# GTEC-UDC/roskfpos

Hardware: AMD Instinct MI355X
Metric: EKF predict+update steps/s at 65536 tags x 8 anchors; RMS pos err vs CPU ref (higher is better)
Workload: dtype f64 arithmetic; f64 state and covariance, f32/int32 measurements in HBM (KFPOS_STORE_MIXED)

## Files before the change

### __graft_entry__.py

```python
from __future__ import annotations

import os
import shutil
import subprocess
import sys

ROOT = os.path.dirname(os.path.abspath(__file__))
CSRC = os.path.join(ROOT, "roskfpos_amd", "csrc")
HIP_LIB = os.path.join(CSRC, "libkfpos_hip.so")
ADAPTOR_DEMO = os.path.join(CSRC, "kfpos_replay")


def _stale(target, sources):
    if not os.path.exists(target):
        return True
    mt = os.path.getmtime(target)
    return any(os.path.getmtime(s) > mt for s in sources if os.path.exists(s))


def build(force: bool = False) -> None:
    jobs = str(min(8, os.cpu_count() or 1))
    res = subprocess.run(["make", "-s", "-j", jobs, "-C", CSRC] + (["-B"] if force else []) + ["all"],
                         capture_output=True, text=True)
    if res.returncode != 0:
        sys.stderr.write(res.stdout + res.stderr)
        raise subprocess.CalledProcessError(res.returncode, res.args)
    res = subprocess.run(["make", "-s", "-C", CSRC, "check"], capture_output=True, text=True)
    if res.returncode != 0:
        sys.stderr.write(res.stdout + res.stderr)
        if os.path.exists(HIP_LIB):
            os.remove(HIP_LIB)
        raise RuntimeError("a build-time performance rule is broken (scratch inside a loop / a kernel lost its second "
                           "wavefront per SIMD / the 9-state epoch loop waits for a memory operation just issued): " + (res.stdout + res.stderr).strip())
    subprocess.check_call(["make", "-s", "-C", os.path.join(ROOT, "oracle")] + (["-B"] if force else []))
    import glob
    core_headers = sorted(glob.glob(os.path.join(CSRC, "kfpos_core*.h"))) + [os.path.join(CSRC, "kfpos_p48.h")]
    emu_dir = os.path.join(ROOT, "tests", "emu")
    emu_so = os.path.join(emu_dir, "libkfpos_emu.so")
    if force or _stale(emu_so, [os.path.join(emu_dir, "kfpos_emu.cpp")] + core_headers):
        subprocess.check_call(["g++", "-O2", "-std=c++17", "-fPIC", "-shared", "-Wno-unknown-pragmas",
                               "-o", emu_so, os.path.join(emu_dir, "kfpos_emu.cpp")])
    fake_dir = os.path.join(ROOT, "tests", "fake_rccl")
    fake_so = os.path.join(fake_dir, "libfake_rccl.so")
    if force or _stale(fake_so, [os.path.join(fake_dir, "fake_rccl.cpp")]):
        subprocess.check_call([shutil.which("hipcc") or "/opt/rocm/bin/hipcc", "-O2", "-std=c++17", "-shared", "-fPIC",
                               "-o", fake_so, os.path.join(fake_dir, "fake_rccl.cpp"), "-lrt"])
    if ROOT not in sys.path:
        sys.path.insert(0, ROOT)
    import roskfpos_amd
    from roskfpos_amd import capi
    capi.load()


def smoke() -> None:
    if ROOT not in sys.path:
        sys.path.insert(0, ROOT)
# ... 34 lines not shown
```

### roskfpos_amd/csrc/kfpos_core.h

```cpp
#ifndef KFPOS_CORE_H
#define KFPOS_CORE_H

#include <math.h>
#include <stdint.h>

#ifndef KFPOS_HD
#define KFPOS_HD
#endif
#define KFPOS_FN KFPOS_HD inline __attribute__((always_inline))
#if defined(__clang__)
#define KFPOS_UNROLL _Pragma("unroll")
#define KFPOS_NOUNROLL _Pragma("nounroll")
#else
#define KFPOS_UNROLL
#define KFPOS_NOUNROLL
#endif

#if defined(__HIP_DEVICE_COMPILE__)
#define KFPOS_WAVE_ALL(pred) (__all((pred) ? 1 : 0) != 0)
#else
#define KFPOS_WAVE_ALL(pred) (pred)
#endif

namespace kfpos {

enum : uint32_t {
    ST_UPDATE_SKIPPED = 0x01u,
    ST_ML_FALLBACK    = 0x02u,
    ST_FEW_RANGES     = 0x04u,
    ST_ML_INIT        = 0x08u,
    ST_NOT_STARTED    = 0x10u,
    ST_NONFINITE      = 0x20u,
    ST_SKIPPED        = 0x40u,
};
enum : uint32_t { FL_STARTED = 1u, FL_HAS_IMU = 2u };

KFPOS_FN uint32_t pack_status(uint32_t flags, int gain_iters, int ml_iters, int ignored) {
    const uint32_t g = gain_iters > 255 ? 255u : (uint32_t)gain_iters;
    const uint32_t m = ml_iters > 255 ? 255u : (uint32_t)ml_iters;
    return flags | (g << 8) | (m << 16) | ((uint32_t)(ignored + 1) << 24);
}

KFPOS_FN double kf_rcp(double x) {
#if defined(__HIP_DEVICE_COMPILE__)
    double y = __builtin_amdgcn_rcp(x);
    double e = __builtin_fma(-x, y, 1.0);
    y = __builtin_fma(y, e, y);
    e = __builtin_fma(-x, y, 1.0);
    return __builtin_fma(y, e, y);
#else
    return 1.0 / x;
#endif
}
KFPOS_FN double kf_fma(double a, double b, double c) {
#if defined(__HIP_DEVICE_COMPILE__)
    return __builtin_fma(a, b, c);
#else
    return a * b + c;
#endif
}
KFPOS_FN int kf_opaque_zero() {
    int z = 0;
#if defined(__HIP_DEVICE_COMPILE__)
    asm volatile("" : "+v"(z));
#endif
    return z;
}
KFPOS_FN int kf_ctz64(uint64_t m) {
#if defined(__HIP_DEVICE_COMPILE__)
    return __ffsll((unsigned long long)m) - 1;
#else
    return __builtin_ctzll(m);
#endif
}
KFPOS_FN double kf_rsqrt(double x) {
#if defined(__HIP_DEVICE_COMPILE__)
    double y = __builtin_amdgcn_rsq(x);
    const double h = 0.5 * x;
    double e = __builtin_fma(-h * y, y, 0.5);
    y = __builtin_fma(y, e, y);
    e = __builtin_fma(-h * y, y, 0.5);
    return __builtin_fma(y, e, y);
#else
    return 1.0 / sqrt(x);
#endif
}
KFPOS_FN void kf_sqrt_rsqrt(double x, double &d, double &invd) {
#if defined(__HIP_DEVICE_COMPILE__)
    invd = kf_rsqrt(x);
    const double s = x * invd;
// ... 14 lines not shown
    invd = y;
#else
    d = sqrt(x);
    invd = 1.0 / d;
#endif
}

KFPOS_FN double kf_mm_to_m(int32_t mm) {
#if defined(__HIP_DEVICE_COMPILE__)
    const double x = (double)mm;
    const double q = x * 0.001;
    const double r = __builtin_fma(-q, 1000.0, x);
    return __builtin_fma(r, 0.001, q);
#else
    return (double)mm / 1000;
#endif
}

KFPOS_FN bool rel_change_below(double cost, double c, double tol) {
    const double lhs = fabs(cost - c), rhs = tol * cost;
    const bool clear = cost > 0.0 && fabs(lhs - rhs) > 1e-13 * rhs;
    if (KFPOS_WAVE_ALL(clear)) return lhs < rhs;
    return lhs / cost < tol;
}

KFPOS_FN bool rel_change_above(double cost, double c, double tol) {
    const double lhs = fabs(cost - c), rhs = tol * cost;
    const bool clear = cost > 0.0 && fabs(lhs - rhs) > 1e-13 * rhs;
    if (KFPOS_WAVE_ALL(clear)) return lhs > rhs;
    return lhs / cost > tol;
}

KFPOS_FN double stdmax(double a, double b) { return (a < b) ? b : a; }

template <int N, bool SYMM>
struct Cov {
    static constexpr int SZ = SYMM ? N * (N + 1) / 2 : N * N;
    double a[SZ];
    KFPOS_HD static constexpr int idx(int i, int j) {
        return SYMM ? (i <= j ? i * N - i * (i - 1) / 2 + (j - i) : j * N - j * (j - 1) / 2 + (i - j))
                    : i * N + j;
    }
    KFPOS_HD double operator()(int i, int j) const { return a[idx(i, j)]; }
    KFPOS_HD double &operator()(int i, int j) { return a[idx(i, j)]; }
};

// ... 252 lines not shown
```

### roskfpos_amd/csrc/kfpos_core_imu9.h

```cpp
#ifndef KFPOS_CORE_IMU9_H
#define KFPOS_CORE_IMU9_H

namespace kfpos {

constexpr double INFO_FORM_MIN_PIVOT = 1e-7;

struct Tag9 {
    double pos[3], vel[3];
    Cov<9, true> P;
};
struct Imu {
    bool has;
    double acc[3];
    double *ci;
    int ci_stride;
    KFPOS_HD double Wi(int k) const { return ci[(6 + k) * ci_stride]; }
};

KFPOS_FN void imu_whitener(const double s[9], double *ci, int ci_stride) {
    double c00, c11, c22, i00, i11, i22;
    kf_sqrt_rsqrt(s[0], c00, i00);
    const double c10 = s[3] * i00, c20 = s[6] * i00;
    kf_sqrt_rsqrt(s[4] - c10 * c10, c11, i11);
    const double c21 = (s[7] - c20 * c10) * i11;
// ... 407 lines not shown
            u0 += gx * yw; u1 += gy * yw; u2 += gz * yw;
            const double wx = w * gx, wy = w * gy, wz = w * gz;
            m0 += wx * gx; m1 += wx * gy; m2 += wx * gz;
            m3 += wy * gy; m4 += wy * gz; m5 += wz * gz;
        });
        s.c = c;
        s.m[0] = m0; s.m[1] = m1; s.m[2] = m2; s.m[3] = m3; s.m[4] = m4; s.m[5] = m5;
        s.u[0] = u0; s.u[1] = u1; s.u[2] = u2;
    }
}

KFPOS_FN void iekf9_spread_reads() {
#if defined(__HIP_DEVICE_COMPILE__)
    KFPOS_UNROLL
    for (int k = 0; k < 20; ++k) {
        __builtin_amdgcn_sched_group_barrier(0x100, 1, 0);
        __builtin_amdgcn_sched_group_barrier(0x002, 10, 0);
    }
#endif
}
struct Iekf9Parked {
    double binv[21], wi[6];
};
template <bool EVERY_TRIP>
KFPOS_FN void iekf9_fetch(const double *binv, int binv_stride, const Imu &imu, Iekf9Parked &pk) {
    const int z = EVERY_TRIP ? kf_opaque_zero() : 0;
    KFPOS_UNROLL
    for (int k = 0; k < 21; ++k) pk.binv[k] = binv[k * binv_stride + z];
    KFPOS_UNROLL
    for (int k = 0; k < 6; ++k) pk.wi[k] = imu.ci[(6 + k) * imu.ci_stride + z];
}
template <bool DIAG>
KFPOS_FN bool iekf9_pass(const double xhat[9], const Iekf9Parked &pk, const Imu &imu, double tol,
                         const Sweep9 &sw, Iekf9Iter &it, Iekf9Out &o) {
    const double *ve = it.ve;
    const double acc[3] = {xhat[6] + ve[3], xhat[7] + ve[4], xhat[8] + ve[5]};
    double c = it.qd + sw.c;
    const double m0 = sw.m[0], m1 = sw.m[1], m2 = sw.m[2], m3 = sw.m[3], m4 = sw.m[4], m5 = sw.m[5];
    const double m[6] = {m0, m1, m2, m3, m4, m5};
    double u[6] = {sw.u[0] + (m0 * ve[0] + m1 * ve[1] + m2 * ve[2]), sw.u[1] + (m1 * ve[0] + m3 * ve[1] + m4 * ve[2]),
                   sw.u[2] + (m2 * ve[0] + m4 * ve[1] + m5 * ve[2]), 0.0, 0.0, 0.0};
    double ma[6] = {0, 0, 0, 0, 0, 0};
    if (imu.has) {
        const double ya[3] = {imu.acc[0] - acc[0], imu.acc[1] - acc[1], imu.acc[2] - acc[2]};
        const double va[3] = {ya[0] + acc[0] * ve[3], ya[1] + acc[1] * ve[4], ya[2] + acc[2] * ve[5]};
        if constexpr (DIAG) {
            const double wd[3] = {pk.wi[0], pk.wi[3], pk.wi[5]};
            KFPOS_UNROLL
            for (int i = 0; i < 3; ++i) {
                const double wy = wd[i] * ya[i];
                c += ya[i] * wy;
                u[3 + i] = acc[i] * (wd[i] * va[i]);
            }
            ma[0] = acc[0] * acc[0] * wd[0]; ma[3] = acc[1] * acc[1] * wd[1]; ma[5] = acc[2] * acc[2] * wd[2];
        } else {
            const double wm[3][3] = {{pk.wi[0], pk.wi[1], pk.wi[2]},
                                     {pk.wi[1], pk.wi[3], pk.wi[4]},
                                     {pk.wi[2], pk.wi[4], pk.wi[5]}};
            KFPOS_UNROLL
            for (int i = 0; i < 3; ++i) {
                const double wy = wm[i][0] * ya[0] + wm[i][1] * ya[1] + wm[i][2] * ya[2];
                c += ya[i] * wy;
                u[3 + i] = acc[i] * (wm[i][0] * va[0] + wm[i][1] * va[1] + wm[i][2] * va[2]);
            }
            ma[0] = acc[0] * acc[0] * wm[0][0]; ma[1] = acc[0] * acc[1] * wm[0][1]; ma[2] = acc[0] * acc[2] * wm[0][2];
            ma[3] = acc[1] * acc[1] * wm[1][1]; ma[4] = acc[1] * acc[2] * wm[1][2]; ma[5] = acc[2] * acc[2] * wm[2][2];
        }
    }
    if (rel_change_below(it.cost, c, tol)) return false;
#ifdef KFPOS_EMU_ITER_TRACE
    kfpos_emu_iter_trace(o.gain_iters, ve, c);
#endif
    it.cost = c;
    KFPOS_UNROLL
    for (int k = 0; k < 6; ++k) o.mrlast[k] = m[k];
    o.dlast[0] = acc[0]; o.dlast[1] = acc[1]; o.dlast[2] = acc[2];

    Cov<6, true> K;
    KFPOS_UNROLL
    for (int k = 0; k < 21; ++k) K.a[k] = pk.binv[k];
    K(0, 0) += m[0]; K(0, 1) += m[1]; K(0, 2) += m[2]; K(1, 1) += m[3]; K(1, 2) += m[4]; K(2, 2) += m[5];
    K(3, 3) += ma[0]; K(4, 4) += ma[3]; K(5, 5) += ma[5];
    if constexpr (!DIAG) { K(3, 4) += ma[1]; K(3, 5) += ma[2]; K(4, 5) += ma[4]; }
    double v[6];
    sym6_solve(K, u, v);
    double *wl = it.wl;
    wl[0] = u[0] - (m[0] * v[0] + m[1] * v[1] + m[2] * v[2]);
    wl[1] = u[1] - (m[1] * v[0] + m[3] * v[1] + m[4] * v[2]);
    wl[2] = u[2] - (m[2] * v[0] + m[4] * v[1] + m[5] * v[2]);
    wl[3] = u[3] - (ma[0] * v[3] + ma[1] * v[4] + ma[2] * v[5]);
    wl[4] = u[4] - (ma[1] * v[3] + ma[3] * v[4] + ma[4] * v[5]);
    wl[5] = u[5] - (ma[2] * v[3] + ma[4] * v[4] + ma[5] * v[5]);
    double qd = 0.0;
    KFPOS_UNROLL
    for (int i = 0; i < 6; ++i) qd += wl[i] * v[i];
    it.qd = qd;
    KFPOS_UNROLL
    for (int i = 0; i < 6; ++i) it.ve[i] = v[i];
    o.gain_iters++;
    return true;
}

#if defined(__HIP_DEVICE_COMPILE__)
KFPOS_FN double lane_pull(double v, int src4) {
    const int lo = __builtin_amdgcn_ds_bpermute(src4, __double2loint(v));
    const int hi = __builtin_amdgcn_ds_bpermute(src4, __double2hiint(v));
    return __hiloint2double(hi, lo);
}
KFPOS_FN int nth_set_bit(uint64_t m, int n) {
    uint32_t w = (uint32_t)m;
    int base = 0;
    const int c0 = __popc(w);
    if (n >= c0) { n -= c0; w = (uint32_t)(m >> 32); base = 32; }
    KFPOS_UNROLL
    for (int width = 16; width >= 1; width >>= 1) {
        const uint32_t low = w & ((1u << width) - 1u);
        const int c = __popc(low);
        if (n >= c) { n -= c; w >>= width; base += width; }
        else w = low;
    }
    return base;
}

// ... 29 lines not shown
    ci.has = __builtin_amdgcn_ds_bpermute(src4, imu.has ? 1 : 0) != 0;
    KFPOS_UNROLL
    for (int k = 0; k < 3; ++k) ci.acc[k] = lane_pull(imu.acc[k], src4);
    ci.ci = imu.ci + (src - lane);
    ci.ci_stride = imu.ci_stride;
    double r4[4], w4[4];
    KFPOS_UNROLL
    for (int k = 0; k < 4; ++k) {
        const double r0 = lane_pull(sc.r[k], src4), r1 = lane_pull(sc.r[4 + k], src4);
        const double w0 = lane_pull(sc.w[k], src4), w1 = lane_pull(sc.w[4 + k], src4);
        r4[k] = h ? r1 : r0;
        w4[k] = h ? w1 : w0;
    }
    const double *cbinv = binv + (src - lane);
    const double *b4 = anchor_tab + 12 * h;
    const double b0[3] = {b4[0], b4[1], b4[2]};
    while (act) {
        double bb[12];
        const int z = kf_opaque_zero();
        bb[0] = b0[0]; bb[1] = b0[1]; bb[2] = b0[2];
        KFPOS_UNROLL
        for (int k = 3; k < 12; ++k) bb[k] = b4[k + z];
        Iekf9Parked pk;
        iekf9_fetch<true>(cbinv, binv_stride, ci, pk);
        const double p[3] = {xh[0] + ct.ve[0], xh[1] + ct.ve[1], xh[2] + ct.ve[2]};
        Sweep9 sw, other;
        iekf9_sweep4(p, r4, w4, bb, sw);
        other.c = dpp_exchange(sw.c, 0);
        KFPOS_UNROLL
        for (int k = 0; k < 6; ++k) other.m[k] = dpp_exchange(sw.m[k], 0);
        KFPOS_UNROLL
        for (int k = 0; k < 3; ++k) other.u[k] = dpp_exchange(sw.u[k], 0);
        sweep9_add(sw, other);
        iekf9_spread_reads();
        const bool more = iekf9_pass<DIAG>(xh, pk, ci, tol, sw, ct, co);
        act = more && co.gain_iters < max_steps;
    }
    const bool owner = (m >> lane) & 1ull;
    const int rank = __popcll(m & ((1ull << lane) - 1ull));
    const int from4 = (owner ? 2 * rank : lane) << 2;
    KFPOS_UNROLL
    for (int k = 0; k < 6; ++k) {
        const double a = lane_pull(ct.wl[k], from4), b = lane_pull(co.mrlast[k], from4);
        if (owner) { it.wl[k] = a; o.mrlast[k] = b; }
    }
    KFPOS_UNROLL
    for (int k = 0; k < 3; ++k) {
        const double a = lane_pull(co.dlast[k], from4);
        if (owner) o.dlast[k] = a;
    }
    const double cst = lane_pull(ct.cost, from4);
    const int gi = __builtin_amdgcn_ds_bpermute(from4, co.gain_iters);
    if (owner) { it.cost = cst; o.gain_iters = gi; }
}
#endif

template <bool DIAG, bool RANGING, bool ACC0 = false, class SC>
KFPOS_FN void iekf9_info(const double xhat[9], const double *binv, int binv_stride, SC &sc, const Params &pr,
                         const Imu &imu, int max_steps, double tol, Iekf9Out &o) {
    Iekf9Iter it;
    KFPOS_UNROLL
    for (int k = 0; k < 6; ++k) { it.ve[k] = 0.0; it.wl[k] = 0.0; o.mrlast[k] = 0.0; }
    it.qd = 0.0;
    it.cost = 1e20;
    o.dlast[0] = o.dlast[1] = o.dlast[2] = 0.0;
    o.gain_iters = 0;
#if defined(__HIP_DEVICE_COMPILE__)
    constexpr bool PAIRS = RANGING && SC::NA == 8 && SC::CHUNK == 0 && !SC::COOP;
    const bool pairs = PAIRS && pr.pair_anchor_tab && __builtin_amdgcn_ballot_w64(true) == ~0ull;
#endif
    bool more = true;
    int stop = max_steps;
#if defined(__HIP_DEVICE_COMPILE__)
    if (pairs) stop = 8 < max_steps ? 8 : max_steps;
#endif
    for (;;) {
        while (more && o.gain_iters < stop) {
            Iekf9Parked pk;
            iekf9_fetch<false>(binv, binv_stride, imu, pk);
            const double p[3] = {xhat[0] + it.ve[0], xhat[1] + it.ve[1], xhat[2] + it.ve[2]};
            Sweep9 sw;
            iekf9_sweep<RANGING>(p, sc, pr, sw);
            more = iekf9_pass<DIAG>(xhat, pk, imu, tol, sw, it, o);
        }
#if defined(__HIP_DEVICE_COMPILE__)
        if constexpr (PAIRS) {
            if (pairs) {
                const uint64_t m = __builtin_amdgcn_ballot_w64(more && o.gain_iters < max_steps);
                if (m == 0) break;
                if (__popcll(m) <= 32) {
                    iekf9_pairs<DIAG, ACC0>(m, xhat, binv, binv_stride, sc, pr.pair_anchor_tab, imu, max_steps, tol, it, o);
                    break;
                }
                stop = stop + 4 < max_steps ? stop + 4 : max_steps;
                continue;
            }
        }
#endif
        break;
    }
    KFPOS_UNROLL
    for (int k = 0; k < 6; ++k) o.w[k] = it.wl[k];
    o.cost = it.cost;
}

KFPOS_FN void cov_update9(Cov<9, true> &P, const double mr[6], const double d[3], const Imu &imu) {
// ... 12 lines not shown
            }
            pt[i] = v;
        }
        KFPOS_UNROLL
        for (int l = 0; l < 6; ++l) {
            const bool nz = (l < 3 && k < 3 && l >= k) || (l >= 3 && k >= 3 && l <= k);
            if (nz) s += L9(f, l, k) * pt[e9(l)];
        }
        const double is = kf_rcp(s);
        KFPOS_UNROLL
        for (int i = 0; i < 9; ++i) {
            const double pi = pt[i] * is;
            KFPOS_UNROLL
            for (int j = i; j < 9; ++j) P(i, j) -= pi * pt[j];
        }
    }
}

struct CovPark9 {
    double *a;
    int stride;
};

template <bool RANGING, class SC>
KFPOS_FN bool step_imu9_state(Tag9 &tg, SC &sc, const Params &pr, double dt, const Imu &imu, const CovPark9 &park,
                              bool diag, Iekf9Out &o, uint32_t &status) {
    constexpr bool has_ranging = RANGING;
    const int n_valid = has_ranging ? count_used(sc, pr, 0) : 0;
    if (!pr.use_init_pos && (isnan(tg.pos[0]) || isnan(tg.pos[1]))) {
        status = 0;
        if (!has_ranging) return false;
        status = ST_FEW_RANGES;
        if (n_valid < 4) return false;
        double p[3] = {1.0, 1.0, 4.0}, sse, c[6];
        set_weights_ml(sc, pr, 0ull);
        const int it = ml_estimate(p, sc, pr, 0, n_valid, sse);
        status = ST_UPDATE_SKIPPED;
        if (ml_covariance_throws(sc, pr, 0, n_valid, sse)) return false;
        if (!ml_covariance(p, sc, pr, sse, c)) return false;
        tg.pos[0] = p[0]; tg.pos[1] = p[1]; tg.pos[2] = p[2];
        tg.P(0, 0) = c[0]; tg.P(0, 1) = c[1]; tg.P(1, 1) = c[3];
        status = pack_status(ST_ML_INIT, 0, it, -1);
        return false;
    }
    const double c = dt * dt / 2;
    double xhat[9];
    KFPOS_UNROLL
    for (int k = 0; k < 3; ++k) {
        xhat[k] = tg.pos[k] + dt * tg.vel[k] + c * 0.0;
        xhat[3 + k] = tg.vel[k] + dt * 0.0;
        xhat[6 + k] = 0.0;
    }
    predict9(tg.P, dt, pr.jolt);
    Cov<6, true> B;
    KFPOS_UNROLL
    for (int i = 0; i < 6; ++i) {
        KFPOS_UNROLL
        for (int j = i; j < 6; ++j) B(i, j) = tg.P(e9(i), e9(j));
    }
    KFPOS_UNROLL
    for (int k = 0; k < 45; ++k) park.a[k * park.stride] = tg.P.a[k];
    double *binv = park.a + 45 * park.stride;
    const bool invertible = sym6_inverse(B, binv, park.stride, INFO_FORM_MIN_PIVOT);
    iekf9_weights(xhat, sc, pr, has_ranging, n_valid, o);
    if (o.flags & ST_UPDATE_SKIPPED) {
        KFPOS_UNROLL
        for (int k = 0; k < 45; ++k) tg.P.a[k] = park.a[k * park.stride];
        status = ST_UPDATE_SKIPPED;
        return false;
    }
    if (invertible) {
        if (diag) iekf9_info<true, RANGING, true>(xhat, binv, park.stride, sc, pr, imu, 20, 1e-4, o);
        else iekf9_info<false, RANGING, true>(xhat, binv, park.stride, sc, pr, imu, 20, 1e-4, o);
        KFPOS_UNROLL
        for (int k = 0; k < 45; ++k) tg.P.a[k] = park.a[k * park.stride];
    } else {
        KFPOS_UNROLL
        for (int k = 0; k < 45; ++k) tg.P.a[k] = park.a[k * park.stride];
        if (diag) iekf9<true, RANGING>(xhat, tg.P, sc, pr, imu, 20, 1e-4, o);
        else iekf9<false, RANGING>(xhat, tg.P, sc, pr, imu, 20, 1e-4, o);
    }
    KFPOS_UNROLL
    for (int i = 0; i < 6; ++i) {
        double v = 0.0;
        KFPOS_UNROLL
        for (int k = 0; k < 6; ++k) v += tg.P(i, e9(k)) * o.w[k];
        if (i < 3) tg.pos[i] = xhat[i] + v;
        else tg.vel[i - 3] = xhat[i] + v;
    }
    status = 0;
    return true;
}
KFPOS_FN uint32_t step_imu9_cov(Tag9 &tg, const Iekf9Out &o, const Imu &imu) {
    cov_update9(tg.P, o.mrlast, o.dlast, imu);
    return pack_status(o.flags, o.gain_iters, o.ml_iters, -1);
}
template <bool RANGING, class SC>
KFPOS_FN uint32_t step_imu9(Tag9 &tg, SC &sc, const Params &pr, double dt, const Imu &imu, const CovPark9 &park) {
    Iekf9Out o;
    uint32_t status;
    if (!step_imu9_state<RANGING>(tg, sc, pr, dt, imu, park, false, o, status)) return status;
    return step_imu9_cov(tg, o, imu);
// ... 22 lines not shown
```

### roskfpos_amd/csrc/kfpos_k_imu9.hip

```cpp
#include "kfpos_kernels.h"

namespace {

template <typename REAL, typename MREAL, int AS, bool RANGING = true>
__global__ __launch_bounds__(WAVE) void k_step_imu9(const KArgs a) {
    extern __shared__ double lds[];
    const int lane = threadIdx.x;
    const size_t t = (size_t)blockIdx.x * WAVE + lane;
    if (t >= (size_t)a.T) return;
    const size_t T = a.T;
    const uint32_t t32 = (uint32_t)t;
    Params pr = make_params(a);
    constexpr bool has_ranging = RANGING;
    constexpr bool AHEAD = sizeof(MREAL) == 4 && !std::is_same<REAL, float>::value;
    const bool fresh_imu = a.mode != MODE_TOA;
    constexpr int NA = AS > 0 ? AS : 1;
    double dt_tag = a.dt_shared;
    if (a.n_steps == 1 && a.dt) {
        dt_tag = a.dt[t32];
        if (dt_tag < 0.0) {
            skipped_lane(a, t, true);
            return;
        }
    }
// ... 33 lines not shown
#pragma unroll
        for (int k = 0; k < 3; ++k) imu.acc[k] = ldrow<MREAL>(a.imu_acc, k, T, t32);
        cv[0] = ldrow<MREAL>(a.imu_cov, 0, T, t32);
        cv[3] = ldrow<MREAL>(a.imu_cov, 1, T, t32);
        cv[4] = ldrow<MREAL>(a.imu_cov, 2, T, t32);
        cv[6] = ldrow<MREAL>(a.imu_cov, 3, T, t32);
        cv[7] = ldrow<MREAL>(a.imu_cov, 4, T, t32);
        cv[8] = ldrow<MREAL>(a.imu_cov, 5, T, t32);
    }
#pragma unroll
    for (int k = 0; k < 45; ++k) tg.P.a[k] = ldcov<REAL>(a.P, k, 45, T, t32);
    if (fresh_imu) {
        imu.has = true;
#pragma unroll
        for (int k = 0; k < 9; ++k) cv[k] = (double)rawc[k];
        if (a.latch) latch_imu_cov<MREAL>(a, T, t32, cv);
    }
    if (imu.has) imu_whitener(cv, imu.ci, imu.ci_stride);
    bool diag = false;
    if (a.imu9_diag) {
        const bool mine = !imu.has || (imu.Wi(1) == 0.0 && imu.Wi(2) == 0.0 && imu.Wi(4) == 0.0);
        diag = __builtin_amdgcn_ballot_w64(mine) == __builtin_amdgcn_ballot_w64(true);
    }

    const bool multi = a.n_steps > 1;
    double dt_next = multi ? a.dt_steps[0] : dt_tag;
    constexpr bool IMU_WITH_EPOCH = AHEAD && AS > 0 && RANGING;

    __builtin_amdgcn_s_waitcnt(0x0F70);
    uint32_t s = 0;
    for (int e = 0; e < a.n_steps; ++e) {
        const double dt = dt_next;
        if (multi && e + 1 < a.n_steps) dt_next = a.dt_steps[opaque_uniform(e + 1)];
        if (fresh_imu) {
#pragma unroll
            for (int k = 0; k < 3; ++k) imu.acc[k] = (double)rawi.acc[k];
            if constexpr (AHEAD && !IMU_WITH_EPOCH) {
                if (e + 1 < a.n_steps) fetch_imu<MREAL>(a, opaque_lane(t), opaque_uniform(e + 1), rawi);
            }
        }
        Iekf9Out o;
        auto finish = [&](bool update) {
            if (a.traj) {
#pragma unroll
                for (int k = 0; k < 3; ++k) (a.traj + ((size_t)opaque_uniform(e) * 3 + k) * T)[t32] = tg.pos[k];
            }
            if (update) s = step_imu9_cov(tg, o, imu);
        };
        if constexpr (AS > 0) {
            RegScratch<AS> sc;
            if (has_ranging) {
                unpack_epoch<MREAL, AS>(raw, sc);
                if (e + 1 < a.n_steps) {
                    if constexpr (AHEAD) {
                        fetch_epoch<MREAL, AS>(a, opaque_lane(t), opaque_uniform(e + 1), raw);
                        if constexpr (IMU_WITH_EPOCH) {
                            if (fresh_imu) fetch_imu<MREAL>(a, opaque_lane(t), opaque_uniform(e + 1), rawi);
                        }
                    }
                }
            } else {
#pragma unroll
                for (int k = 0; k < AS; ++k) sc.r[k] = sc.e[k] = sc.w[k] = 0.0;
            }
            finish(step_imu9_state<RANGING>(tg, sc, pr, dt, imu, park, diag, o, s));
            if constexpr (!AHEAD) {
                if (e + 1 < a.n_steps) {
                    if (fresh_imu) fetch_imu<MREAL>(a, opaque_lane(t), opaque_uniform(e + 1), rawi);
                    if (has_ranging) fetch_epoch<MREAL, AS>(a, opaque_lane(t), opaque_uniform(e + 1), raw);
                }
            }
        } else {
            Scratch sc{nullptr, nullptr, nullptr, WAVE};
            if (has_ranging) sc = stage_epoch_lds<MREAL>(a, lds, lane, t, opaque_uniform(e));
            finish(step_imu9_state<RANGING>(tg, sc, pr, dt, imu, park, diag, o, s));
            if constexpr (!AHEAD) {
                if (e + 1 < a.n_steps && fresh_imu) fetch_imu<MREAL>(a, opaque_lane(t), opaque_uniform(e + 1), rawi);
            }
        }
        if constexpr (cov_is_rounded<REAL>()) {
            if (e + 1 < a.n_steps) {
#pragma unroll
                for (int k = 0; k < 45; ++k) tg.P.a[k] = round_cov<REAL>(tg.P.a[k]);
            }
        }
    }

    if (fresh_imu && a.latch) {
#pragma unroll
        for (int k = 0; k < 3; ++k) strow<MREAL>(a.imu_acc, k, T, t32, imu.acc[k]);
        fl |= FL_HAS_IMU;
    }
    bool fin = true;
#pragma unroll
    for (int k = 0; k < 3; ++k) {
        (a.pos + k * T)[t32] = tg.pos[k];
        (a.vel + k * T)[t32] = tg.vel[k];
        fin &= isfinite(tg.pos[k]) & isfinite(tg.vel[k]);
// ... 24 lines not shown
```

### roskfpos_amd/csrc/kfpos_k_imu9each.hip

```cpp
#include "kfpos_kernels.h"

namespace {

template <typename REAL, typename MREAL, int AS>
__global__ __launch_bounds__(WAVE) void k_events_imu9_each(const kfpos_k::EvEachArgs ev) {
    extern __shared__ double lds[];
    const KArgs &a = ev.k;
    const int lane = threadIdx.x;
    const size_t t = (size_t)blockIdx.x * WAVE + lane;
    if (t >= (size_t)a.T) return;
    const size_t T = a.T;
    const uint32_t t32 = (uint32_t)t;
    const Params pr = make_params(a);
    constexpr bool AHEAD = sizeof(MREAL) == 4 && !std::is_same<REAL, float>::value;
    constexpr int NA = AS > 0 ? AS : 1;
    const int n = a.n_steps;
    auto is_toa = [&](int e) -> int { return opaque_uniform((int)((ev.kinds[(e >> 6) & 1] >> (e & 63)) & 1ull)); };
    auto load_dt = [&](int e) -> double { return (ev.dt_each + (size_t)e * T)[(uint32_t)opaque_lane(t)]; };

    uint32_t fl = a.flags[t32];
    double dt_next = load_dt(0);
    RawEpoch<MREAL, NA> raw;
    RawImu<MREAL> rawi;
    int toa = is_toa(0);
// ... 75 lines not shown
            }
        };
        const bool run = !(dt < 0.0);
        const bool last_status = !more && a.status;
        if (__builtin_amdgcn_ballot_w64(run) == 0) {
            fetch_small();
            fetch_epoch_next();
            if (a.traj) {
#pragma unroll
                for (int k = 0; k < 3; ++k) (a.traj + ((size_t)opaque_uniform(e) * 3 + k) * T)[t32] = tg.pos[k];
            }
            if (ev.status_events) (ev.status_events + (size_t)opaque_uniform(e) * T)[t32] = ST_SKIPPED;
            if (last_status) a.status[t32] = ST_SKIPPED;
            toa = toa_next;
            continue;
        }
        Iekf9Out o;
        bool update = false;
        if (toa) {
            if constexpr (AS > 0) {
                RegScratch<AS> sc;
                unpack_epoch<MREAL, AS>(raw, sc);
                if constexpr (AHEAD) fetch_small();
                if (run) update = step_imu9_state<true>(tg, sc, pr, dt, imu, park, diag, o, s);
            } else {
                Scratch sc = stage_epoch_lds<MREAL>(a, lds, lane, t, opaque_uniform(cur));
                if constexpr (AHEAD) fetch_small();
                if (run) update = step_imu9_state<true>(tg, sc, pr, dt, imu, park, diag, o, s);
            }
        } else {
            if (run) {
#pragma unroll
                for (int k = 0; k < 3; ++k) imu.acc[k] = (double)rawi.acc[k];
                imu.has = true;
                if (!ci_is_cov) {
                    MREAL rc[9];
                    fetch_imu_cov<MREAL>(a, opaque_lane(t), 0, rc);
                    double cv[9];
#pragma unroll
                    for (int k = 0; k < 9; ++k) cv[k] = (double)rc[k];
                    imu_whitener(cv, imu.ci, imu.ci_stride);
                    ci_is_cov = true;
                }
                sampled = true;
            }
            if constexpr (AHEAD) fetch_small();
            Scratch sc{nullptr, nullptr, nullptr, WAVE};
            if (run) update = step_imu9_state<false>(tg, sc, pr, dt, imu, park, diag, o, s);
        }
        ran |= run;
        if (a.traj) {
#pragma unroll
            for (int k = 0; k < 3; ++k) (a.traj + ((size_t)opaque_uniform(e) * 3 + k) * T)[t32] = tg.pos[k];
        }
        if (update) s = step_imu9_cov(tg, o, imu);
        if constexpr (!AHEAD) fetch_small();
        fetch_epoch_next();
        if (ev.status_events || last_status) {
            uint32_t w = ST_SKIPPED;
            if (run) {
                bool fin = true;
#pragma unroll
                for (int k = 0; k < 3; ++k) fin &= isfinite(tg.pos[k]) & isfinite(tg.vel[k]);
#pragma unroll
                for (int k = 0; k < 45; ++k) fin &= isfinite(tg.P.a[k]);
                const bool waiting = !a.use_init_pos && isnan(tg.pos[0]);
                w = (!fin && !waiting) ? (s | ST_NONFINITE) : s;
            }
            if (ev.status_events) (ev.status_events + (size_t)opaque_uniform(e) * T)[t32] = w;
            if (last_status) a.status[t32] = w;
        }
// ... 41 lines not shown
```

### roskfpos_amd/csrc/kfpos_k_imu9ev.hip

```cpp
#include "kfpos_kernels.h"

namespace {

template <typename REAL, typename MREAL, int AS>
__global__ __launch_bounds__(WAVE) void k_events_imu9(const kfpos_k::EvArgs ev) {
    extern __shared__ double lds[];
    const KArgs &a = ev.k;
    const int lane = threadIdx.x;
    const size_t t = (size_t)blockIdx.x * WAVE + lane;
    if (t >= (size_t)a.T) return;
    const size_t T = a.T;
    const uint32_t t32 = (uint32_t)t;
    const Params pr = make_params(a);
    constexpr bool AHEAD = sizeof(MREAL) == 4 && !std::is_same<REAL, float>::value;
    constexpr int NA = AS > 0 ? AS : 1;
    const int n = a.n_steps;
    auto is_toa = [&](int e) -> int { return opaque_uniform((int)((ev.kinds[(e >> 6) & 1] >> (e & 63)) & 1ull)); };

    uint32_t fl = a.flags[t32];
    RawEpoch<MREAL, NA> raw;
    RawImu<MREAL> rawi;
    int toa = is_toa(0);
    if (toa) {
        if constexpr (AS > 0) fetch_epoch<MREAL, AS>(a, t, 0, raw);
// ... 6 lines not shown
        tg.pos[k] = (a.pos + k * T)[t32];
        tg.vel[k] = (a.vel + k * T)[t32];
    }
    const CovPark9 park{lds + (AS == 0 ? 3 * (size_t)a.A * WAVE : 0) + lane, WAVE};
    Imu imu;
    imu.ci = park.a + 66 * WAVE;
    imu.ci_stride = WAVE;
    MREAL rawc[9];
    fetch_imu_cov<MREAL>(a, t, 0, rawc);
    imu.has = (fl & FL_HAS_IMU) != 0;
    if (imu.has) {
#pragma unroll
        for (int k = 0; k < 3; ++k) imu.acc[k] = ldrow<MREAL>(a.imu_acc, k, T, t32);
    } else {
#pragma unroll
        for (int k = 0; k < 3; ++k) imu.acc[k] = 0.0;
    }
#pragma unroll
    for (int k = 0; k < 45; ++k) tg.P.a[k] = ldcov<REAL>(a.P, k, 45, T, t32);
    double cv[9];
#pragma unroll
    for (int k = 0; k < 9; ++k) cv[k] = (double)rawc[k];
    imu_whitener(cv, imu.ci, imu.ci_stride);
    bool diag = false;
    if (a.imu9_diag) {
        const bool mine = imu.Wi(1) == 0.0 && imu.Wi(2) == 0.0 && imu.Wi(4) == 0.0;
        diag = __builtin_amdgcn_ballot_w64(mine) == __builtin_amdgcn_ballot_w64(true);
    }

    double dt_next = a.dt_steps[0];
    __builtin_amdgcn_s_waitcnt(0x0F70);
    uint32_t s = 0;
    int it = 0, ii = 0;
    int sampled = 0;
    for (int e = 0; e < n; ++e) {
        const double dt = dt_next;
        const bool more = e + 1 < n;
        int toa_next = 0;
        if (more) {
            dt_next = a.dt_steps[opaque_uniform(e + 1)];
            toa_next = is_toa(opaque_uniform(e + 1));
        }
        const int mine = it;
        (void)mine;
        it += toa;
        ii += 1 - toa;
        auto fetch_next = [&]() {
            if (!more) return;
            if (toa_next) {
                if constexpr (AS > 0) fetch_epoch<MREAL, AS>(a, opaque_lane(t), opaque_uniform(it), raw);
            } else {
                fetch_imu<MREAL>(a, opaque_lane(t), opaque_uniform(ii), rawi);
            }
        };
        Iekf9Out o;
        bool update;
        if (toa) {
            if constexpr (AS > 0) {
                RegScratch<AS> sc;
                unpack_epoch<MREAL, AS>(raw, sc);
                if constexpr (AHEAD) fetch_next();
                update = step_imu9_state<true>(tg, sc, pr, dt, imu, park, diag, o, s);
            } else {
                Scratch sc = stage_epoch_lds<MREAL>(a, lds, lane, t, opaque_uniform(mine));
                if constexpr (AHEAD) fetch_next();
                update = step_imu9_state<true>(tg, sc, pr, dt, imu, park, diag, o, s);
            }
        } else {
#pragma unroll
            for (int k = 0; k < 3; ++k) imu.acc[k] = (double)rawi.acc[k];
            imu.has = true;
            sampled = 1;
            if constexpr (AHEAD) fetch_next();
            Scratch sc{nullptr, nullptr, nullptr, WAVE};
            update = step_imu9_state<false>(tg, sc, pr, dt, imu, park, diag, o, s);
        }
        if (a.traj) {
#pragma unroll
            for (int k = 0; k < 3; ++k) (a.traj + ((size_t)opaque_uniform(e) * 3 + k) * T)[t32] = tg.pos[k];
        }
        if (update) s = step_imu9_cov(tg, o, imu);
        if constexpr (!AHEAD) fetch_next();
        if (ev.status_events && more) {
            bool fin = true;
#pragma unroll
            for (int k = 0; k < 3; ++k) fin &= isfinite(tg.pos[k]) & isfinite(tg.vel[k]);
#pragma unroll
            for (int k = 0; k < 45; ++k) fin &= isfinite(tg.P.a[k]);
            const bool waiting = !a.use_init_pos && isnan(tg.pos[0]);
            (ev.status_events + (size_t)opaque_uniform(e) * T)[t32] = (!fin && !waiting) ? (s | ST_NONFINITE) : s;
        }
        if constexpr (cov_is_rounded<REAL>()) {
            if (more) {
#pragma unroll
                for (int k = 0; k < 45; ++k) tg.P.a[k] = round_cov<REAL>(tg.P.a[k]);
            }
        }
        toa = toa_next;
// ... 41 lines not shown
```

### roskfpos_amd/csrc/kfpos_kernels.h

```cpp
#ifndef KFPOS_KERNELS_H
#define KFPOS_KERNELS_H

#include <hip/hip_runtime.h>

#include <cmath>
#include <cstdint>
#include <type_traits>

#define KFPOS_HD __host__ __device__
#include "kfpos_core.h"
#include "kfpos_internal.h"
#include "kfpos_p48.h"

namespace kfpos_k {

struct KArgs {
    double anchors[KFPOS_MAX_ANCHORS * 3];
    int T, A;
    double accel_noise, jolt, cost_threshold;
    int ignore_worst, top_n, use_init_pos, ml_variant;
    int pair9;
    int imu9_diag;
    int use_fixed_height, imu_fixed_cov_acc, imu_fixed_cov_w;
    double px4_height, px4_arm_p1, px4_arm_p2, px4_cov_vel, px4_cov_gyro_z;
// ... 283 lines not shown
};
template <typename MREAL>
__device__ inline void fetch_imu(const KArgs &a, size_t t, int s, RawImu<MREAL> &raw) {
    const MREAL *ap = (const MREAL *)a.accel + (size_t)s * a.stride_accel;
#pragma unroll
    for (int k = 0; k < 3; ++k) raw.acc[k] = (ap + (size_t)k * a.T)[(uint32_t)t];
}
template <typename MREAL>
__device__ inline void fetch_imu_cov(const KArgs &a, size_t t, int s, MREAL raw[9]) {
    const MREAL *cp = (const MREAL *)a.cov + (size_t)s * a.stride_cov;
#pragma unroll
    for (int k = 0; k < 9; ++k) raw[k] = (cp + (size_t)k * a.T)[(uint32_t)t];
}
template <typename MREAL>
__device__ inline void latch_imu_cov(const KArgs &a, size_t T, uint32_t t32, const double cv[9]) {
    strow<MREAL>(a.imu_cov, 0, T, t32, cv[0]);
    strow<MREAL>(a.imu_cov, 1, T, t32, cv[3]);
    strow<MREAL>(a.imu_cov, 2, T, t32, cv[4]);
    strow<MREAL>(a.imu_cov, 3, T, t32, cv[6]);
    strow<MREAL>(a.imu_cov, 4, T, t32, cv[7]);
    strow<MREAL>(a.imu_cov, 5, T, t32, cv[8]);
}

__device__ inline int opaque_uniform(int v) {
    asm volatile("" : "+s"(v));
    return v;
}
__device__ inline size_t opaque_lane(size_t t) {
    uint32_t v = (uint32_t)t;
    asm volatile("" : "+v"(v));
    return v;
}
template <int N>
__device__ inline StaticScratchF<N> stage_epoch_lds_nf(const KArgs &a, double *lds, int lane, size_t t, int s) {
    StaticScratchF<N> sc;
    sc.r = lds + lane;
    sc.w = lds + (size_t)N * WAVE + lane;
    sc.e = (float *)(lds + 2 * (size_t)N * WAVE) + lane;
    sc.stride = WAVE;
    RawEpoch<float, N> raw;
    fetch_epoch<float, N>(a, t, s, raw);
#pragma unroll
    for (int k = 0; k < N; ++k) {
        sc.r[k * WAVE] = raw.mm[k] > 0 ? kf_mm_to_m(raw.mm[k]) : 0.0;
        sc.e[k * WAVE] = raw.e[k];
    }
// ... 20 lines not shown
```

Before: 2.021 billion.

## Hoist parked IEKF9 loads out of gain loop and streamline per-trip convergence vote

The parked inverse-covariance and IMU whitener values are now fetched once before the 9-state information-form gain iteration instead of on every trip, and the whitener entries are pinned in registers. The convergence test now assumes the fast comparison and only falls back to a division when some lane votes it is unclear. The pass body becomes predicated rather than early-returning. A wave-uniform 'fast' path is added that skips the per-lane IMU-presence branch when every lane has IMU data and a diagonal whitener. The hoist is disabled for the f64/f32/8-anchor events kernel, presumably to limit register pressure there. Holding values in registers across the loop can raise VGPR use and threaten occupancy in the kernels that keep it enabled.

```diff
diff --git a/__graft_entry__.py b/__graft_entry__.py
--- a/__graft_entry__.py
+++ b/__graft_entry__.py
@@ -31,7 +31,8 @@
         if os.path.exists(HIP_LIB):
             os.remove(HIP_LIB)
         raise RuntimeError("a build-time performance rule is broken (scratch inside a loop / a kernel lost its second "
-                           "wavefront per SIMD / the 9-state epoch loop waits for a memory operation just issued): " + (res.stdout + res.stderr).strip())
+                           "wavefront per SIMD / the 9-state epoch loop waits for a memory operation just issued / a trip of its gain "
+                           "iteration touches memory or branches too often): " + (res.stdout + res.stderr).strip())
     subprocess.check_call(["make", "-s", "-C", os.path.join(ROOT, "oracle")] + (["-B"] if force else []))
     import glob
     core_headers = sorted(glob.glob(os.path.join(CSRC, "kfpos_core*.h"))) + [os.path.join(CSRC, "kfpos_p48.h")]
diff --git a/roskfpos_amd/csrc/kfpos_core.h b/roskfpos_amd/csrc/kfpos_core.h
--- a/roskfpos_amd/csrc/kfpos_core.h
+++ b/roskfpos_amd/csrc/kfpos_core.h
@@ -20,6 +20,11 @@
 #define KFPOS_WAVE_ALL(pred) (__all((pred) ? 1 : 0) != 0)
 #else
 #define KFPOS_WAVE_ALL(pred) (pred)
+#endif
+#if defined(__HIP_DEVICE_COMPILE__)
+#define KFPOS_WAVE_ANY(pred) (__builtin_amdgcn_ballot_w64(pred) != 0)
+#else
+#define KFPOS_WAVE_ANY(pred) (pred)
 #endif
 
 namespace kfpos {
@@ -66,6 +71,13 @@
 #endif
     return z;
 }
+KFPOS_FN void kf_pin(double &v) {
+#if defined(__HIP_DEVICE_COMPILE__)
+    asm volatile("" : "+v"(v));
+#else
+    (void)v;
+#endif
+}
 KFPOS_FN int kf_ctz64(uint64_t m) {
 #if defined(__HIP_DEVICE_COMPILE__)
     return __ffsll((unsigned long long)m) - 1;
@@ -126,6 +138,14 @@
     const bool clear = cost > 0.0 && fabs(lhs - rhs) > 1e-13 * rhs;
     if (KFPOS_WAVE_ALL(clear)) return lhs < rhs;
     return lhs / cost < tol;
+}
+
+KFPOS_FN bool rel_change_below_voted(double cost, double c, double tol) {
+    const double lhs = fabs(cost - c), rhs = tol * cost;
+    const bool clear = cost > 0.0 && fabs(lhs - rhs) > 1e-13 * rhs;
+    bool below = lhs < rhs;
+    if (KFPOS_WAVE_ANY(!clear)) below = lhs / cost < tol;
+    return below;
 }
 
 KFPOS_FN bool rel_change_above(double cost, double c, double tol) {
diff --git a/roskfpos_amd/csrc/kfpos_core_imu9.h b/roskfpos_amd/csrc/kfpos_core_imu9.h
--- a/roskfpos_amd/csrc/kfpos_core_imu9.h
+++ b/roskfpos_amd/csrc/kfpos_core_imu9.h
@@ -453,15 +453,21 @@
 struct Iekf9Parked {
     double binv[21], wi[6];
 };
-template <bool EVERY_TRIP>
+template <bool EVERY_TRIP, bool DIAG, bool PIN = !EVERY_TRIP>
 KFPOS_FN void iekf9_fetch(const double *binv, int binv_stride, const Imu &imu, Iekf9Parked &pk) {
     const int z = EVERY_TRIP ? kf_opaque_zero() : 0;
     KFPOS_UNROLL
     for (int k = 0; k < 21; ++k) pk.binv[k] = binv[k * binv_stride + z];
     KFPOS_UNROLL
     for (int k = 0; k < 6; ++k) pk.wi[k] = imu.ci[(6 + k) * imu.ci_stride + z];
-}
-template <bool DIAG>
+    if constexpr (PIN) {
+        KFPOS_UNROLL
+        for (int k = 0; k < 6; ++k) {
+            if (!DIAG || k == 0 || k == 3 || k == 5) kf_pin(pk.wi[k]);
+        }
+    }
+}
+template <bool DIAG, bool ALLIMU>
 KFPOS_FN bool iekf9_pass(const double xhat[9], const Iekf9Parked &pk, const Imu &imu, double tol,
                          const Sweep9 &sw, Iekf9Iter &it, Iekf9Out &o) {
     const double *ve = it.ve;
@@ -472,7 +478,7 @@
     double u[6] = {sw.u[0] + (m0 * ve[0] + m1 * ve[1] + m2 * ve[2]), sw.u[1] + (m1 * ve[0] + m3 * ve[1] + m4 * ve[2]),
                    sw.u[2] + (m2 * ve[0] + m4 * ve[1] + m5 * ve[2]), 0.0, 0.0, 0.0};
     double ma[6] = {0, 0, 0, 0, 0, 0};
-    if (imu.has) {
+    if (ALLIMU || imu.has) {
         const double ya[3] = {imu.acc[0] - acc[0], imu.acc[1] - acc[1], imu.acc[2] - acc[2]};
         const double va[3] = {ya[0] + acc[0] * ve[3], ya[1] + acc[1] * ve[4], ya[2] + acc[2] * ve[5]};
         if constexpr (DIAG) {
@@ -498,38 +504,40 @@
             ma[3] = acc[1] * acc[1] * wm[1][1]; ma[4] = acc[1] * acc[2] * wm[1][2]; ma[5] = acc[2] * acc[2] * wm[2][2];
         }
     }
-    if (rel_change_below(it.cost, c, tol)) return false;
+    const bool go = !rel_change_below_voted(it.cost, c, tol);
+    if (go) {
 #ifdef KFPOS_EMU_ITER_TRACE
-    kfpos_emu_iter_trace(o.gain_iters, ve, c);
+        kfpos_emu_iter_trace(o.gain_iters, ve, c);
 #endif
-    it.cost = c;
-    KFPOS_UNROLL
-    for (int k = 0; k < 6; ++k) o.mrlast[k] = m[k];
-    o.dlast[0] = acc[0]; o.dlast[1] = acc[1]; o.dlast[2] = acc[2];
-
-    Cov<6, true> K;
-    KFPOS_UNROLL
-    for (int k = 0; k < 21; ++k) K.a[k] = pk.binv[k];
-    K(0, 0) += m[0]; K(0, 1) += m[1]; K(0, 2) += m[2]; K(1, 1) += m[3]; K(1, 2) += m[4]; K(2, 2) += m[5];
-    K(3, 3) += ma[0]; K(4, 4) += ma[3]; K(5, 5) += ma[5];
-    if constexpr (!DIAG) { K(3, 4) += ma[1]; K(3, 5) += ma[2]; K(4, 5) += ma[4]; }
-    double v[6];
-    sym6_solve(K, u, v);
-    double *wl = it.wl;
-    wl[0] = u[0] - (m[0] * v[0] + m[1] * v[1] + m[2] * v[2]);
-    wl[1] = u[1] - (m[1] * v[0] + m[3] * v[1] + m[4] * v[2]);
-    wl[2] = u[2] - (m[2] * v[0] + m[4] * v[1] + m[5] * v[2]);
-    wl[3] = u[3] - (ma[0] * v[3] + ma[1] * v[4] + ma[2] * v[5]);
-    wl[4] = u[4] - (ma[1] * v[3] + ma[3] * v[4] + ma[4] * v[5]);
-    wl[5] = u[5] - (ma[2] * v[3] + ma[4] * v[4] + ma[5] * v[5]);
-    double qd = 0.0;
-    KFPOS_UNROLL
-    for (int i = 0; i < 6; ++i) qd += wl[i] * v[i];
-    it.qd = qd;
-    KFPOS_UNROLL
-    for (int i = 0; i < 6; ++i) it.ve[i] = v[i];
-    o.gain_iters++;
-    return true;
+        it.cost = c;
+        KFPOS_UNROLL
+        for (int k = 0; k < 6; ++k) o.mrlast[k] = m[k];
+        o.dlast[0] = acc[0]; o.dlast[1] = acc[1]; o.dlast[2] = acc[2];
+
+        Cov<6, true> K;
+        KFPOS_UNROLL
+        for (int k = 0; k < 21; ++k) K.a[k] = pk.binv[k];
+        K(0, 0) += m[0]; K(0, 1) += m[1]; K(0, 2) += m[2]; K(1, 1) += m[3]; K(1, 2) += m[4]; K(2, 2) += m[5];
+        K(3, 3) += ma[0]; K(4, 4) += ma[3]; K(5, 5) += ma[5];
+        if constexpr (!DIAG) { K(3, 4) += ma[1]; K(3, 5) += ma[2]; K(4, 5) += ma[4]; }
+        double v[6];
+        sym6_solve(K, u, v);
+        double *wl = it.wl;
+        wl[0] = u[0] - (m[0] * v[0] + m[1] * v[1] + m[2] * v[2]);
+        wl[1] = u[1] - (m[1] * v[0] + m[3] * v[1] + m[4] * v[2]);
+        wl[2] = u[2] - (m[2] * v[0] + m[4] * v[1] + m[5] * v[2]);
+        wl[3] = u[3] - (ma[0] * v[3] + ma[1] * v[4] + ma[2] * v[5]);
+        wl[4] = u[4] - (ma[1] * v[3] + ma[3] * v[4] + ma[4] * v[5]);
+        wl[5] = u[5] - (ma[2] * v[3] + ma[4] * v[4] + ma[5] * v[5]);
+        double qd = 0.0;
+        KFPOS_UNROLL
+        for (int i = 0; i < 6; ++i) qd += wl[i] * v[i];
+        it.qd = qd;
+        KFPOS_UNROLL
+        for (int i = 0; i < 6; ++i) it.ve[i] = v[i];
+        o.gain_iters++;
+    }
+    return go;
 }
 
 #if defined(__HIP_DEVICE_COMPILE__)
@@ -605,7 +613,7 @@
         KFPOS_UNROLL
         for (int k = 3; k < 12; ++k) bb[k] = b4[k + z];
         Iekf9Parked pk;
-        iekf9_fetch<true>(cbinv, binv_stride, ci, pk);
+        iekf9_fetch<true, DIAG>(cbinv, binv_stride, ci, pk);
         const double p[3] = {xh[0] + ct.ve[0], xh[1] + ct.ve[1], xh[2] + ct.ve[2]};
         Sweep9 sw, other;
         iekf9_sweep4(p, r4, w4, bb, sw);
@@ -616,7 +624,7 @@
         for (int k = 0; k < 3; ++k) other.u[k] = dpp_exchange(sw.u[k], 0);
         sweep9_add(sw, other);
         iekf9_spread_reads();
-        const bool more = iekf9_pass<DIAG>(xh, pk, ci, tol, sw, ct, co);
+        const bool more = iekf9_pass<DIAG, false>(xh, pk, ci, tol, sw, ct, co);
         act = more && co.gain_iters < max_steps;
     }
     const bool owner = (m >> lane) & 1ull;
@@ -638,7 +646,7 @@
 }
 #endif
 
-template <bool DIAG, bool RANGING, bool ACC0 = false, class SC>
+template <bool DIAG, bool ALLIMU, bool RANGING, bool ACC0 = false, bool HOLD = true, class SC>
 KFPOS_FN void iekf9_info(const double xhat[9], const double *binv, int binv_stride, SC &sc, const Params &pr,
                          const Imu &imu, int max_steps, double tol, Iekf9Out &o) {
     Iekf9Iter it;
@@ -657,14 +665,15 @@
 #if defined(__HIP_DEVICE_COMPILE__)
     if (pairs) stop = 8 < max_steps ? 8 : max_steps;
 #endif
+    Iekf9Parked pk;
+    if constexpr (HOLD) iekf9_fetch<false, DIAG, true>(binv, binv_stride, imu, pk);
     for (;;) {
         while (more && o.gain_iters < stop) {
-            Iekf9Parked pk;
-            iekf9_fetch<false>(binv, binv_stride, imu, pk);
+            if constexpr (!HOLD) iekf9_fetch<false, DIAG, false>(binv, binv_stride, imu, pk);
             const double p[3] = {xhat[0] + it.ve[0], xhat[1] + it.ve[1], xhat[2] + it.ve[2]};
             Sweep9 sw;
             iekf9_sweep<RANGING>(p, sc, pr, sw);
-            more = iekf9_pass<DIAG>(xhat, pk, imu, tol, sw, it, o);
+            more = iekf9_pass<DIAG, ALLIMU>(xhat, pk, imu, tol, sw, it, o);
         }
 #if defined(__HIP_DEVICE_COMPILE__)
         if constexpr (PAIRS) {
@@ -723,9 +732,9 @@
     int stride;
 };
 
-template <bool RANGING, class SC>
+template <bool RANGING, bool HOLD = true, class SC>
 KFPOS_FN bool step_imu9_state(Tag9 &tg, SC &sc, const Params &pr, double dt, const Imu &imu, const CovPark9 &park,
-                              bool diag, Iekf9Out &o, uint32_t &status) {
+                              bool fast, Iekf9Out &o, uint32_t &status) {
     constexpr bool has_ranging = RANGING;
     const int n_valid = has_ranging ? count_used(sc, pr, 0) : 0;
     if (!pr.use_init_pos && (isnan(tg.pos[0]) || isnan(tg.pos[1]))) {
@@ -771,14 +780,14 @@
         return false;
     }
     if (invertible) {
-        if (diag) iekf9_info<true, RANGING, true>(xhat, binv, park.stride, sc, pr, imu, 20, 1e-4, o);
-        else iekf9_info<false, RANGING, true>(xhat, binv, park.stride, sc, pr, imu, 20, 1e-4, o);
+        if (fast) iekf9_info<true, true, RANGING, true, HOLD>(xhat, binv, park.stride, sc, pr, imu, 20, 1e-4, o);
+        else iekf9_info<false, false, RANGING, true, HOLD>(xhat, binv, park.stride, sc, pr, imu, 20, 1e-4, o);
         KFPOS_UNROLL
         for (int k = 0; k < 45; ++k) tg.P.a[k] = park.a[k * park.stride];
     } else {
         KFPOS_UNROLL
         for (int k = 0; k < 45; ++k) tg.P.a[k] = park.a[k * park.stride];
-        if (diag) iekf9<true, RANGING>(xhat, tg.P, sc, pr, imu, 20, 1e-4, o);
+        if (fast) iekf9<true, RANGING>(xhat, tg.P, sc, pr, imu, 20, 1e-4, o);
         else iekf9<false, RANGING>(xhat, tg.P, sc, pr, imu, 20, 1e-4, o);
     }
     KFPOS_UNROLL
diff --git a/roskfpos_amd/csrc/kfpos_k_imu9.hip b/roskfpos_amd/csrc/kfpos_k_imu9.hip
--- a/roskfpos_amd/csrc/kfpos_k_imu9.hip
+++ b/roskfpos_amd/csrc/kfpos_k_imu9.hip
@@ -79,6 +79,7 @@
         const bool mine = !imu.has || (imu.Wi(1) == 0.0 && imu.Wi(2) == 0.0 && imu.Wi(4) == 0.0);
         diag = __builtin_amdgcn_ballot_w64(mine) == __builtin_amdgcn_ballot_w64(true);
     }
+    const bool fast = imu9_fast(diag, imu.has);
 
     const bool multi = a.n_steps > 1;
     double dt_next = multi ? a.dt_steps[0] : dt_tag;
@@ -120,7 +121,7 @@
 #pragma unroll
                 for (int k = 0; k < AS; ++k) sc.r[k] = sc.e[k] = sc.w[k] = 0.0;
             }
-            finish(step_imu9_state<RANGING>(tg, sc, pr, dt, imu, park, diag, o, s));
+            finish(step_imu9_state<RANGING>(tg, sc, pr, dt, imu, park, fast, o, s));
             if constexpr (!AHEAD) {
                 if (e + 1 < a.n_steps) {
                     if (fresh_imu) fetch_imu<MREAL>(a, opaque_lane(t), opaque_uniform(e + 1), rawi);
@@ -130,7 +131,7 @@
         } else {
             Scratch sc{nullptr, nullptr, nullptr, WAVE};
             if (has_ranging) sc = stage_epoch_lds<MREAL>(a, lds, lane, t, opaque_uniform(e));
-            finish(step_imu9_state<RANGING>(tg, sc, pr, dt, imu, park, diag, o, s));
+            finish(step_imu9_state<RANGING>(tg, sc, pr, dt, imu, park, fast, o, s));
             if constexpr (!AHEAD) {
                 if (e + 1 < a.n_steps && fresh_imu) fetch_imu<MREAL>(a, opaque_lane(t), opaque_uniform(e + 1), rawi);
             }
diff --git a/roskfpos_amd/csrc/kfpos_k_imu9each.hip b/roskfpos_amd/csrc/kfpos_k_imu9each.hip
--- a/roskfpos_amd/csrc/kfpos_k_imu9each.hip
+++ b/roskfpos_amd/csrc/kfpos_k_imu9each.hip
@@ -121,11 +121,11 @@
                 RegScratch<AS> sc;
                 unpack_epoch<MREAL, AS>(raw, sc);
                 if constexpr (AHEAD) fetch_small();
-                if (run) update = step_imu9_state<true>(tg, sc, pr, dt, imu, park, diag, o, s);
+                if (run) update = step_imu9_state<true>(tg, sc, pr, dt, imu, park, imu9_fast(diag, imu.has), o, s);
             } else {
                 Scratch sc = stage_epoch_lds<MREAL>(a, lds, lane, t, opaque_uniform(cur));
                 if constexpr (AHEAD) fetch_small();
-                if (run) update = step_imu9_state<true>(tg, sc, pr, dt, imu, park, diag, o, s);
+                if (run) update = step_imu9_state<true>(tg, sc, pr, dt, imu, park, imu9_fast(diag, imu.has), o, s);
             }
         } else {
             if (run) {
@@ -145,7 +145,7 @@
             }
             if constexpr (AHEAD) fetch_small();
             Scratch sc{nullptr, nullptr, nullptr, WAVE};
-            if (run) update = step_imu9_state<false>(tg, sc, pr, dt, imu, park, diag, o, s);
+            if (run) update = step_imu9_state<false>(tg, sc, pr, dt, imu, park, imu9_fast(diag, imu.has), o, s);
         }
         ran |= run;
         if (a.traj) {
diff --git a/roskfpos_amd/csrc/kfpos_k_imu9ev.hip b/roskfpos_amd/csrc/kfpos_k_imu9ev.hip
--- a/roskfpos_amd/csrc/kfpos_k_imu9ev.hip
+++ b/roskfpos_amd/csrc/kfpos_k_imu9ev.hip
@@ -52,6 +52,7 @@
 #pragma unroll
     for (int k = 0; k < 9; ++k) cv[k] = (double)rawc[k];
     imu_whitener(cv, imu.ci, imu.ci_stride);
+    constexpr bool HOLD = !(std::is_same<REAL, double>::value && sizeof(MREAL) == 4 && AS == 8);
     bool diag = false;
     if (a.imu9_diag) {
         const bool mine = imu.Wi(1) == 0.0 && imu.Wi(2) == 0.0 && imu.Wi(4) == 0.0;
@@ -90,11 +91,11 @@
                 RegScratch<AS> sc;
                 unpack_epoch<MREAL, AS>(raw, sc);
                 if constexpr (AHEAD) fetch_next();
-                update = step_imu9_state<true>(tg, sc, pr, dt, imu, park, diag, o, s);
+                update = step_imu9_state<true, HOLD>(tg, sc, pr, dt, imu, park, imu9_fast(diag, imu.has), o, s);
             } else {
                 Scratch sc = stage_epoch_lds<MREAL>(a, lds, lane, t, opaque_uniform(mine));
                 if constexpr (AHEAD) fetch_next();
-                update = step_imu9_state<true>(tg, sc, pr, dt, imu, park, diag, o, s);
+                update = step_imu9_state<true, HOLD>(tg, sc, pr, dt, imu, park, imu9_fast(diag, imu.has), o, s);
             }
         } else {
 #pragma unroll
@@ -103,7 +104,7 @@
             sampled = 1;
             if constexpr (AHEAD) fetch_next();
             Scratch sc{nullptr, nullptr, nullptr, WAVE};
-            update = step_imu9_state<false>(tg, sc, pr, dt, imu, park, diag, o, s);
+            update = step_imu9_state<false, HOLD>(tg, sc, pr, dt, imu, park, imu9_fast(diag, imu.has), o, s);
         }
         if (a.traj) {
 #pragma unroll
diff --git a/roskfpos_amd/csrc/kfpos_kernels.h b/roskfpos_amd/csrc/kfpos_kernels.h
--- a/roskfpos_amd/csrc/kfpos_kernels.h
+++ b/roskfpos_amd/csrc/kfpos_kernels.h
@@ -329,6 +329,9 @@
     strow<MREAL>(a.imu_cov, 5, T, t32, cv[8]);
 }
 
+__device__ inline bool imu9_fast(bool diag, bool has) {
+    return diag && __builtin_amdgcn_ballot_w64(!has) == 0;
+}
 __device__ inline int opaque_uniform(int v) {
     asm volatile("" : "+s"(v));
     return v;
```

Measured after the change: 2.105 billion, median of 6. +4.2%, better.
